# GadGadGad/Convolutional-KAN-for-Image-Classification

Measured on AMD Instinct MI355X. Metric: images/sec fwd+bwd KAN-VGG11 3x32x32 bs=256/GPU, higher is better.
Workload: dtype f32

## Files before the change

convolutional-kan-for-image-classification_amd/_lib.py:

```python
from __future__ import annotations

import ctypes as C
import os
from typing import Optional

_HERE = os.path.dirname(os.path.abspath(__file__))
LIB_PATH = os.environ.get("KANCONV_LIB") or os.path.join(_HERE, "libkanconv.so")

KAN_MAX_PLANES = 16
KAN_MAX_TABLE = 32
KAN_FP_WORDS = 192
BASIS_BSPLINE, BASIS_RBF, BASIS_CHEBY, BASIS_POLY, BASIS_FOURIER, BASIS_RELU, BASIS_GRAM = 0, 1, 2, 3, 4, 5, 6
ACT_NONE, ACT_IDENTITY, ACT_GELU, ACT_SILU, ACT_RELU, ACT_TANH, ACT_SIGMOID, ACT_GELU_TANH = -1, 0, 1, 2, 3, 4, 5, 6


class KanGeom(C.Structure):
    _fields_ = [(n, C.c_int) for n in ("B", "C", "H", "W", "O", "Ho", "Wo", "kh", "kw", "sh", "sw", "ph", "pw", "dh", "dw", "groups")] + \
               [("x_bstride", C.c_longlong), ("y_bstride", C.c_longlong)]


class KanBasis(C.Structure):
    _fields_ = [("kind", C.c_int), ("n_basis", C.c_int), ("order", C.c_int), ("act", C.c_int),
                ("p0", C.c_float), ("p1", C.c_float), ("table", C.c_float * KAN_MAX_TABLE), ("chan_table", C.c_void_p)]


class KanPlan(C.Structure):
    _fields_ = [(n, C.c_int) for n in ("P", "K", "IPC", "KC", "Kpad", "Opad", "fwd_splits", "bwd_data_splits", "bwd_weight_splits",
                                          "fwd_target", "bwd_data_target", "bwd_weight_target", "x_pm_wanted", "dz_pm_wanted", "bwd_weight_expanded", "row_blocks", "e_pm_wanted", "fwd_expanded", "fwd_halo", "bwd_weight_halo",
                                          "fwd_band", "bwd_weight_band")] + \
               [(n, C.c_longlong) for n in ("packed_weight_bytes", "bwd_data_weight_bytes", "fwd_slab_elems", "bwd_data_slab_elems",
                                            "bwd_weight_slab_elems", "e_pm_elems")]


class KanWavGeom(C.Structure):
    _fields_ = [(n, C.c_int) for n in ("B", "C", "H", "W", "O", "Ho", "Wo", "kh", "kw", "sh", "sw", "ph", "pw", "dh", "dw", "wavelet")] + \
               [("x_bstride", C.c_longlong), ("u_bstride", C.c_longlong)]


WAVELETS = {"mexican_hat": 0, "morlet": 1, "dog": 2, "meyer": 3, "shannon": 4}

_P, _I, _LL, _F, _D = C.c_void_p, C.c_int, C.c_longlong, C.c_float, C.c_double
_GP, _BP = C.POINTER(KanGeom), C.POINTER(KanBasis)
SIGNATURES = {
    "kan_version": (C.c_char_p, []),
    "kan_last_error": (C.c_char_p, []),
    "kan_plan": (_I, [_GP, _BP, C.POINTER(KanPlan)]),
    "kan_pack_weights": (_I, [_P, _P, _P, _P, _GP, _BP, _P]),
    "kan_pack_cacheable": (_I, [_GP, _BP]),
    "kan_pack_weights_cached": (_I, [_P, _P, _P, _P, _GP, _BP, _P, _I, _I, _I, _P]),
    "kan_conv_fwd": (_I, [_P, _P, _P, _P, _GP, _BP, _P, _P]),
    "kan_position_major": (_I, [_P, _P, _I, _I, _I, _LL, _P]),
    "kan_conv_bwd_data": (_I, [_P, _P, _P, _P, _P, _P, _GP, _BP, _P, _P]),
    "kan_conv_bwd_data_params": (_I, [_P, _P, _P, _P, _P, _P, _P, _GP, _BP, _P, _P]),
    "kan_conv_bwd_weight": (_I, [_P, _P, _P, _P, _GP, _BP, _P, _P, _P]),
    "kan_position_major_expanded": (_I, [_P, _P, _GP, _BP, _P]),
    "kan_conv_fwd_expanded": (_I, [_P, _P, _P, _GP, _BP, _P]),
    "kan_conv_bwd_weight_expanded": (_I, [_P, _P, _P, _GP, _BP, _P]),
    "kan_unpack_wgrad": (_I, [_P, _P, _P, _GP, _BP, _P]),
    "kan_slab_reduce": (_I, [_P, _I, _LL, _P, _I, _I, _I, _LL, _P]),
    "kan_instnorm_prelu_fwd": (_I, [_P, _I, _LL, _P, _P, _P, _P, _P, _P, _P, _I, _I, _I, _LL, _F, _I, _P]),
    "kan_instnorm_prelu_bwd": (_I, [_P, _P, _P, _P, _P, _P, _P, _P, _P, _P, _P, _I, _I, _I, _LL, _I, _P]),
    "kan_instnorm_prelu_pool_fwd": (_I, [_P, _I, _LL, _P, _P, _P, _P, _P, _P, _P, _P, _I, _I, _I, _I, _LL, _F, _I, _P]),
    "kan_instnorm_prelu_pool_bwd": (_I, [_P, _P, _P, _P, _P, _P, _P, _P, _P, _P, _P, _P, _I, _I, _I, _I, _LL, _I, _P]),
    "kan_instnorm_prelu_poolk_fwd": (_I, [_P, _I, _LL, _P, _P, _P, _P, _P, _P, _P, _P, _I, _I, _I, _I, _LL, _F, _I, _I, _I, _P]),
    "kan_instnorm_prelu_poolk_bwd": (_I, [_P, _P, _P, _P, _P, _P, _P, _P, _P, _P, _P, _P, _I, _I, _I, _I, _LL, _I, _I, _I, _P]),
    "kan_split_supported": (_I, [C.POINTER(KanGeom), C.POINTER(KanBasis)]),
    "kan_split_weight_bytes": (_LL, [C.POINTER(KanGeom), C.POINTER(KanBasis)]),
    "kan_split_pack_weights": (_I, [_P, _P, _P, C.POINTER(KanGeom), C.POINTER(KanBasis), _P]),
    "kan_conv_fwd_split": (_I, [_P, _P, _P, C.POINTER(KanGeom), C.POINTER(KanBasis), _P]),
    "kan_wav_fwd": (_I, [_P, _P, _P, _P, _P, C.POINTER(KanWavGeom), _P]),
    "kan_wav_bwd_input": (_I, [_P, _P, _P, _P, _P, _P, C.POINTER(KanWavGeom), _P]),
    "kan_wav_param_workspace": (_LL, [C.POINTER(KanWavGeom)]),
    "kan_wav_bwd_params": (_I, [_P, _P, _P, _P, _P, _P, _P, _P, _P, C.POINTER(KanWavGeom), _P]),
    "kan_adamw_step": (_I, [_P, _P, _P, _P, _LL, _D, _D, _D, _D, _D, _I, _F, _P]),
    "kan_adamw_step_segments": (_I, [_P, _P, _P, _P, _P, _P, _P, _P, _P, _I, _I, _D, _D, _D, _D, _D, _I, _F, _P]),
}

_lib: Optional[C.CDLL] = None

# ... 29 lines not shown
```

convolutional-kan-for-image-classification_amd/csrc/kanconv.hip:

```cpp
#include <hip/hip_runtime.h>
#include <cstdio>
#include <cstdlib>
#include <cstring>
#include <cmath>
#include <cstdint>
#include <type_traits>
#include "kanconv.h"
#include "kan_device.h"

#include "kan_common.h"
#include "kan_internal.h"

namespace {


thread_local char g_err[512] = "";
int fail(const char* fmt, const char* a = "") {
    snprintf(g_err, sizeof(g_err), fmt, a);
    return -1;
}
}
int kan_fail_msg(const char* fmt, const char* a) { return fail(fmt, a); }
namespace {

// ... 539 lines not shown
        for (int mi = 0; mi < 2; ++mi) {
#pragma unroll
            for (int r = 0; r < 16; ++r) {
                const int o = o_tile0 + w_o * 64 + mi * 32 + mfma_row(r, lane);
                if (o < g.O) zb[(size_t)o * HoWo] = acc[mi][ni][r];
            }
        }
    }
}

template <int M>
__device__ __forceinline__ void wave_reduce_scatter(float (&v)[M], int lane, int& idx, float& tot) {
    int base = 0;
    int m = M;
#pragma unroll
    for (int off = 32; off >= 1; off >>= 1) {
        if (m > 1) {
            const int h = m / 2;
            const bool up = (lane & off) != 0;
#pragma unroll
            for (int i = 0; i < M / 2; ++i) {
                if (i < h) {
                    const float keep = up ? v[h + i] : v[i], send = up ? v[i] : v[h + i];
                    v[i] = keep + __shfl_xor(send, off, 64);
                }
            }
            base += up ? h : 0;
            m = h;
        } else {
            v[0] += __shfl_xor(v[0], off, 64);
        }
    }
    idx = base; tot = v[0];
}

template <int KIND, int FAST, int RB = 0>
__global__ __launch_bounds__(256, 4) void k_conv_bwd_data(
    const float* __restrict__ dz, const float* __restrict__ x, const float* __restrict__ xn, const float* __restrict__ wd,
    float* __restrict__ dx, float* __restrict__ dxn, DevGeom g, DevBasis bs, int CH, int n_ct, int n_ob, int Opad16,
    int n_chunks, int chunks_per_split, long long slab_elems, unsigned dz_bytes, TilePerm perm, float* __restrict__ dpar) {
    constexpr int TP = 128, KD = 16, NT = 256;
    __shared__ __attribute__((aligned(16))) float smem[2 * 2 * KD * 128];
    __shared__ float sTab[KAN_MAX_TABLE];

    const int tid = threadIdx.x, lane = tid & 63;
    const int wave = __builtin_amdgcn_readfirstlane(tid >> 6);
    const int w_r = wave >> 1, w_p = wave & 1;
    const int HoWo = g.Ho * g.Wo, HW = g.H * g.W, P = bs.P;
    const int Min = g.B * HW;
    const BlockId blk = xcd_block_order(false);
    const int grp = blk.y / n_ct;
    const int px_tile0 = (perm.n ? (int)perm.idx[blk.x] : blk.x) * TP, ct = blk.y - grp * n_ct;
    const int ncol = n_ct * 128;
    const int pxl = (wave & 1) * 64 + lane, ol0 = wave >> 1;
    const bool idle_rows = (ct * 2 + w_r) * CH >= g.C;
    {
        const size_t xo = (size_t)grp * g.C * HW;
        x += xo; xn += xo; dx += xo; if (dxn) dxn += xo;
        dz += (size_t)grp * g.O * HoWo * (g.pix_major ? g.B : 1);
        wd += (size_t)grp * (g.kh * g.kw) * Opad16 * ncol;
    }

    if (tid < KAN_MAX_TABLE) sTab[tid] = bs.tab[tid];
    const int my_px = px_tile0 + (RB ? ((pxl >> 2) & 7) * 16 + (pxl >> 5) * 4 + (pxl & 3) : pxl);
    const bool pv = my_px < Min;
    int pb, ph_, pw_;
// ... 266 lines not shown
#pragma unroll
            for (int it = 0; it < NIT; ++it) {
                if (!((ok >> (half * NIT + it)) & 1u)) continue;
                const int cl = ol0 + 2 * it, c = (ct * 2 + half) * FCH + cl;
                const float xa = half == 0 ? xv[0][it] : xv[1][it];
                float dact;
                if (bs.act == KAN_ACT_SILU) {
                    const float sg = kan_rcp(1.0f + kan_exp2k(xa, -1.44269504088896340736f));
                    dact = sg * (1.0f + xa * (1.0f - sg));
                } else dact = kan_act_grad(bs.act, xa);
                float t = xa, chain = 1.0f;
                if (bs.order) {
                    t = kan_tanh_fast(xa);
                    chain = 1.0f - t * t;
                }
                const float* G = smem + (cl * FP) * TP + pxl;
                float Tm = bs.tab[0], Tc = bs.tab[1] * t + bs.tab[2], Dm = 0.f, Dc = bs.tab[1];
                float sb = 0.f;
#pragma unroll
                for (int k = 1; k < NB; ++k) {
                    sb += Dc * G[(1 + k) * TP];
                    if (k + 1 < NB) {
                        const float A = bs.tab[3 * k], B = bs.tab[3 * k + 1], Cc = bs.tab[3 * k + 2], sc = A * t + B;
                        const float Tn = sc * Tc + Cc * Tm, Dn = A * Tc + sc * Dc + Cc * Dm;
                        Tm = Tc; Tc = Tn; Dm = Dc; Dc = Dn;
                    }
                }
                dxs[(size_t)pb * g.xbs + (size_t)c * HW + (size_t)(ph_ * g.W + pw_)] = dact * G[0] + sb * chain;
            }
        }
        return;
    }
    if (FAST != 0) {
        constexpr int FP = 9, FCH = 7, NIT = (FCH + 1) / 2;
        float xv[2][NIT]; unsigned ok = 0;
#pragma unroll
        for (int half = 0; half < 2; ++half)
#pragma unroll
            for (int it = 0; it < NIT; ++it) {
                const int cl = ol0 + 2 * it, c = (ct * 2 + half) * FCH + cl;
                const bool v = cl < FCH && c < g.C && pv;
                xv[half][it] = v ? x[(size_t)pb * g.xbs + (size_t)c * HW + (size_t)(ph_ * g.W + pw_)] : 0.f;
                ok |= (v ? 1u : 0u) << (half * NIT + it);
            }
        const float hh = 0.5f * bs.inv_h;
#pragma unroll 1
        for (int half = 0; half < 2; ++half) {
            __syncthreads();
            if (w_r == half) {
#pragma unroll
                for (int mi = 0; mi < 2; ++mi)
#pragma unroll
                    for (int ni = 0; ni < 2; ++ni)
#pragma unroll
                        for (int r = 0; r < 16; ++r)
                            smem[(mi * 32 + mfma_row(r, lane)) * TP + w_p * 64 + ni * 32 + (lane & 31)] = acc[mi][ni][r];
            }
            __syncthreads();
#pragma unroll
            for (int it = 0; it < NIT; ++it) {
                if (!((ok >> (half * NIT + it)) & 1u)) continue;
                const int cl = ol0 + 2 * it, c = (ct * 2 + half) * FCH + cl;
                const float xa = half == 0 ? xv[0][it] : xv[1][it];
                float dact;
                if (FAST == 1) {
                    const float sg = kan_rcp(1.0f + kan_exp2k(xa, -1.44269504088896340736f));
                    dact = sg * (1.0f + xa * (1.0f - sg));
                } else dact = kan_act_grad(KAN_ACT_GELU, xa);
                const float* G = smem + (cl * FP) * TP + pxl;
                float sum = dact * G[0];
                if (xa >= bs.g0 && xa < bs.gN) {
                    const int i = min((int)((xa - bs.g0) * bs.inv_h), 10);
#ifdef KAN_EXACT_TRANSCENDENTALS
                    const double ihd = 1.0 / ((double)sTab[i + 1] - (double)sTab[i]), hd = 0.5 * ihd;
                    const double ud = fmin(fmax(((double)xa - (double)sTab[i]) * ihd, 0.0), 1.0), vd = 1.0 - ud, ud2 = ud * ud;
                    const float n0 = (float)(-hd * vd * vd), n1 = (float)(hd * (3.0 * ud2 - 4.0 * ud)), n2 = (float)(hd * (-3.0 * ud2 + 2.0 * ud + 1.0)), n3 = (float)(hd * ud2);
#else
                    const float u = fminf(fmaxf((xa - sTab[i]) * bs.inv_h, 0.f), 1.f), v = 1.f - u, u2 = u * u;
                    const float n0 = -hh * v * v, n1 = hh * (3.f * u2 - 4.f * u), n2 = hh * (-3.f * u2 + 2.f * u + 1.f), n3 = hh * u2;
#endif
                    const int j0 = i - 3;
                    sum += ((unsigned)j0 < 8u ? n0 * G[(1 + j0) * TP] : 0.f) + ((unsigned)(j0 + 1) < 8u ? n1 * G[(2 + j0) * TP] : 0.f)
                         + ((unsigned)(j0 + 2) < 8u ? n2 * G[(3 + j0) * TP] : 0.f) + ((unsigned)(j0 + 3) < 8u ? n3 * G[(4 + j0) * TP] : 0.f);
                }
                dxs[(size_t)pb * g.xbs + (size_t)c * HW + (size_t)(ph_ * g.W + pw_)] = sum;
            }
        }
        return;
    }
#pragma unroll 1
    for (int half = 0; half < 2; ++half) {
        __syncthreads();
        if (w_r == half) {
#pragma unroll
            for (int mi = 0; mi < 2; ++mi)
#pragma unroll
                for (int ni = 0; ni < 2; ++ni)
#pragma unroll
                    for (int r = 0; r < 16; ++r) {
                        int row = mi * 32 + mfma_row(r, lane);
                        int col = w_p * 64 + ni * 32 + (lane & 31);
                        smem[row * TP + col] = acc[mi][ni][r];
                    }
        }
        __syncthreads();
        for (int cl = ol0; cl < CH; cl += 2) {
            const int c = (ct * 2 + half) * CH + cl;
            if (c >= g.C || !pv) continue;
            const size_t idx = (size_t)pb * g.xbs + (size_t)c * HW + (size_t)(ph_ * g.W + pw_);
            const float xa = x[idx];
            const float xb = same_in ? xa : xn[idx];
            float s_base = 0.f, s_bas = 0.f;
            const float* Gc = smem + (cl * P) * TP + pxl;
            kan_planes_each<KIND, true>(bs, sTab, xa, xb, c, [&](int p, float d) {
                const float gv = Gc[p * TP];
                if (p < bs.hb) s_base += d * gv; else s_bas += d * gv;
            });
            if (split_out) { dxs[idx] = s_base; dxns[idx] = s_bas; }
            else dxs[idx] = s_base + s_bas;
        }
// ... 25 lines not shown
                const float xb = pv ? (same_in ? x : xn)[(size_t)pb * g.xbs + (size_t)c * HW + (size_t)(ph_ * g.W + pw_)] : 0.f;
                const float* lo = bs.ctab + (size_t)c * 2 * nb;
                if (2 * nb <= 16) {
                    float v[16];
#pragma unroll
                    for (int j = 0; j < 8; ++j) {
                        float vlo = 0.f, vhi = 0.f;
                        if (j < nb) {
                            const float gv = pv ? smem[(cl * P + hb + j) * TP + pxl] : 0.f;
                            const float x1 = fmaxf(xb - lo[j], 0.f), x2 = fmaxf(lo[nb + j] - xb, 0.f);
                            const float q2 = 2.0f * (x1 * x2 * rr) * rr;
                            vlo = -(q2 * x2) * gv; vhi = (q2 * x1) * gv;
                        }
                        v[j] = vlo; v[8 + j] = vhi;
                    }
                    int idx; float tot;
                    wave_reduce_scatter<16>(v, lane, idx, tot);
                    const int j = idx & 7;
                    if ((lane & 3) == 0 && j < nb) atomicAdd(dpar + (size_t)c * 2 * nb + (idx < 8 ? j : nb + j), tot);
                } else {
                    for (int j = 0; j < nb; ++j) {
                        const float gv = pv ? smem[(cl * P + hb + j) * TP + pxl] : 0.f;
                        const float x1 = fmaxf(xb - lo[j], 0.f), x2 = fmaxf(lo[nb + j] - xb, 0.f);
                        const float q2 = 2.0f * (x1 * x2 * rr) * rr;
                        float vlo = -(q2 * x2) * gv, vhi = (q2 * x1) * gv;
#pragma unroll
                        for (int off = 32; off > 0; off >>= 1) { vlo += __shfl_xor(vlo, off, 64); vhi += __shfl_xor(vhi, off, 64); }
                        if (lane == 0) { atomicAdd(dpar + (size_t)c * 2 * nb + j, vlo); atomicAdd(dpar + (size_t)c * 2 * nb + nb + j, vhi); }
                    }
                }
            }
        }
    }
}

template <int KIND, int FAST, int WR, int WC>
__global__ __launch_bounds__(WR * WC * 64, (WR * WC > 4 ? 2 : 4)) void k_conv_bwd_weight(
    const float* __restrict__ dz, const float* __restrict__ x, const float* __restrict__ xn, float* __restrict__ dwp,
    DevGeom g, DevBasis bs, int Krows, int Opad, int n_chunks, int chunks_per_split, long long slab_elems,
    unsigned x_bytes, unsigned dz_bytes, int tiles_o) {
    constexpr int TR = WR * 64, TO = WC * 64, NT = WR * WC * 64, KPX = 16;
    constexpr int MRG = KAN_PMAX;
    constexpr int LDE = TR + 2 * MRG + 1, LDZ = TO + 1;
    constexpr int IPP = NT / KPX;
    constexpr int UPF = TR / 128;
    constexpr int ZL = TO * KPX / NT;
    constexpr int MAXI = TR + 2;
    __shared__ float sE[2 * KPX * LDE];
    __shared__ float sZ[2 * KPX * LDZ];
    __shared__ int sItem[MAXI];
    __shared__ float sTab[KAN_MAX_TABLE];
    __shared__ float sDump[NT];

    const int tid = threadIdx.x, lane = tid & 63;
    const int wave = __builtin_amdgcn_readfirstlane(tid >> 6);
    const int w_r = wave / WC, w_c = wave % WC;
    const int HoWo = g.Ho * g.Wo, HW = g.H * g.W, T = g.kh * g.kw, P = FAST ? fast_planes(FAST) : bs.P;
    const int Mtot = g.B * HoWo, NI = g.C * T;
    const BlockId blk = xcd_block_order(!g.pix_major);
    const int grp = blk.y / tiles_o;
    const int k0 = blk.x * TR, o_tile0 = (blk.y - grp * tiles_o) * TO;
    {
        const int es = g.pix_major ? g.B : 1;
        const size_t xo = (size_t)grp * g.C * HW * es;
        x += xo; xn += xo;
        dz += (size_t)grp * g.O * HoWo * es;
// ... 1371 lines not shown
        if (best_cost < 0 || cost < best_cost) { best_cost = cost; best = t; best_ms = ms; }
    }
    *max_splits = best_ms;
    return best;
}
int live_taps_out(const KanGeom* g, int hw) {
    int n = 0;
    for (int tap = 0; tap < g->kh * g->kw; ++tap) {
        const int r = tap / g->kw, t = tap % g->kw, ho = hw / g->Wo, wo = hw % g->Wo;
        const int hi = ho * g->sh - g->ph + r * g->dh, wi = wo * g->sw - g->pw + t * g->dw;
        n += (hi >= 0 && hi < g->H && wi >= 0 && wi < g->W);
    }
    return n;
}
int live_taps_in(const KanGeom* g, int hw) {
    int n = 0;
    for (int tap = 0; tap < g->kh * g->kw; ++tap) {
        const int r = tap / g->kw, t = tap % g->kw, h = hw / g->W, w = hw % g->W;
        const int hn = h + g->ph - r * g->dh, wn = w + g->pw - t * g->dw;
        n += (hn >= 0 && wn >= 0 && hn % g->sh == 0 && wn % g->sw == 0 && hn / g->sh < g->Ho && wn / g->sw < g->Wo);
    }
    return n;
}
int live_positions_for_tap(const KanGeom* g, int tap) {
    int n = 0;
    for (int hw = 0; hw < g->Ho * g->Wo; ++hw) {
        const int r = tap / g->kw, t = tap % g->kw, ho = hw / g->Wo, wo = hw % g->Wo;
        const int hi = ho * g->sh - g->ph + r * g->dh, wi = wo * g->sw - g->pw + t * g->dw;
        n += (hi >= 0 && hi < g->H && wi >= 0 && wi < g->W);
    }
    return n;
}
struct BdCfg { int CH, tiles_c, tiles_p, n_ob, Opad32, chunks, splits; };
BdCfg bd_cfg(const KanGeom* g, const KanPlan& pl) {
    BdCfg c;
    c.CH = 64 / pl.P;
    c.tiles_c = ceil_div(g->C, 2 * c.CH);
    c.tiles_p = ceil_div((long long)g->B * g->H * g->W, 128);
    c.n_ob = ceil_div(g->O, 16);
    c.Opad32 = round_up(g->O, 32);
    c.chunks = g->kh * g->kw * c.n_ob;
    c.splits = pick_splits((long long)c.tiles_c * c.tiles_p * ngroups(g), c.chunks, 8, 4.0 * g->B * g->C * g->H * g->W * ngroups(g));
    return c;
}
bool pmdma_bwd_weight(const KanGeom* g, const KanBasis* b) {
    const int f = fast_variant(b);
    if (tuning_off("KAN_PMDMA") || !(f == 1 || f == 2 || f == 9 || f == 10)) return false;
    if (!want_pix_major(g, b, PM_BWD_WEIGHT)) return false;
    const int P = b->n_basis + (b->act != KAN_ACT_NONE);
    return (g->C * P) % 128 == 0 && g->B % 16 == 0 && round_up(g->O, 64) % 128 == 0 &&
           (long long)g->C * g->H * g->W * P * g->B * 4 < (1ll << 31);
}
bool pmdma_fwd(const KanGeom* g, const KanBasis* b) { return pmdma_fwd_shape(g, b) && want_pix_major(g, b, PM_FWD); }
bool halo_bwd_weight(const KanGeom* g, const KanBasis* b) {
    const int f = fast_variant(b);
    if (tuning_off("KAN_HALO_BW") || !(f == 1 || f == 2 || f == 9 || f == 10)) return false;
    if (g->kh != 3 || g->kw != 3 || g->sh != 1 || g->sw != 1 || g->dh != 1 || g->dw != 1 || g->ph != 1 || g->pw != 1) return false;
    if (round_up(g->O, 64) % 128 != 0 || g->C > 65535 / 81) return false;
    if (g->H != g->W) return false;
    if (g->W == 4) return !pmdma_bwd_weight(g, b) && g->B % 2 == 0 && g->C <= 256;
    return g->W == 16 || g->W == 8;
}
bool pm_bwd_weight(const KanGeom* g, const KanBasis* b) { return want_pix_major(g, b, PM_BWD_WEIGHT) && !halo_bwd_weight(g, b); }
struct BwHaloCfg { int R, nimg, spb, n_bands, tiles_r, tiles_o, splits, bands_per_split; };
BwHaloCfg bw_halo_cfg(const KanGeom* g, const KanPlan& pl) {
    BwHaloCfg c;
    c.R = g->W == 16 ? 4 : g->W;
    c.nimg = g->W == 4 ? 2 : 1;
    c.spb = c.nimg * c.R * g->W / 16;
    c.n_bands = g->B * (g->H / c.R) / c.nimg;
    c.tiles_r = ceil_div(pl.K, 128);
    c.tiles_o = pl.Opad / 128;
    const long long tiles = (long long)c.tiles_r * c.tiles_o * ngroups(g);
    const double slab_bytes = 4.0 * pl.K * pl.Opad * ngroups(g);
    int best = 1; double best_cost = -1;
// ... 27 lines not shown
    return !off && g->C == 1 && g->O <= 2 && T <= DW_T && T * P <= DW_MAX_TP;
}
int dw_weight_chunks(const KanGeom* g) {
    const long long total = (long long)g->B * g->Ho * g->Wo;
    int s = ceil_div(2048, ngroups(g));
    const int most = ceil_div(total, 256);
    if (s > most) s = most;
    if (s > 64) s = 64;
    return s < 1 ? 1 : s;
}

int make_plan(const KanGeom* g, const KanBasis* b, KanPlan* pl) {
    if (int rc = check(g, b)) return rc;
    const int T = g->kh * g->kw;
    pl->P = b->n_basis + (b->act != KAN_ACT_NONE);
    pl->K = g->C * T * pl->P;
    {
        int i18 = 18 / pl->P, i16 = 16 / pl->P;
        if (i18 > 4) i18 = 4;
        if (i16 > 4) i16 = 4;
        const bool use18 = (long long)i18 * pl->P * 16 > (long long)i16 * pl->P * 18;
        pl->KC = use18 ? 18 : 16;
        pl->IPC = use18 ? i18 : i16;
        if (pl->P >= 10 && pl->P <= 12) { pl->KC = 12; pl->IPC = 1; }
        if (halo_fwd(g, b)) { pl->KC = 2 * pl->P; pl->IPC = 2; }
    }
    pl->Kpad = ceil_div(g->C * T, pl->IPC) * pl->KC;
    KanBandCfg band;
    const bool use_band = band_fwd(g, b, &band);
    if (use_band) { pl->KC = band.NPLE; pl->IPC = band.NG; pl->Kpad = band.n_steps * band.NPLE; }
    pl->Opad = round_up(g->O, 64);
    const int G = ngroups(g);
    pl->packed_weight_bytes = (long long)G * pl->Kpad * pl->Opad * 4;
    BdCfg bd = bd_cfg(g, *pl);
    pl->bwd_data_weight_bytes = (long long)G * T * bd.Opad32 * bd.tiles_c * 128 * 4;
    pl->fwd_slab_elems = (long long)g->B * g->y_bstride;
    pl->bwd_data_slab_elems = (long long)g->B * g->x_bstride;
    pl->bwd_weight_slab_elems = (long long)G * pl->K * pl->Opad;
    pl->fwd_splits = use_band ? band.fwd_splits : fwd_cfg(g, b, *pl).splits;
    pl->fwd_band = use_band ? 1 : 0;
    pl->bwd_weight_band = (use_band && band.bw_ok && !want_pix_major(g, b, PM_BWD_WEIGHT) && !tuning_off("KAN_BAND_BW")) ? 1 : 0;
    pl->bwd_data_splits = bd.splits;
    pl->bwd_weight_splits = halo_bwd_weight(g, b) ? bw_halo_cfg(g, *pl).splits : bw_cfg(g, b, *pl).splits;
    if (pl->bwd_weight_band) {
        pl->bwd_weight_splits = band.bw_splits;
        pl->bwd_weight_slab_elems = (long long)G * pl->Kpad * pl->Opad;
    }
    pl->x_pm_wanted = ((want_pix_major(g, b, PM_FWD) && !pmdma_fwd(g, b)) || (pm_bwd_weight(g, b) && !pmdma_bwd_weight(g, b))) ? 1 : 0;
    pl->dz_pm_wanted = (want_pix_major(g, b, PM_BWD_DATA) || pm_bwd_weight(g, b)) ? 1 : 0;
    pl->fwd_target = pl->bwd_data_target = pl->bwd_weight_target = 0;
    pl->fwd_halo = halo_fwd(g, b) ? 1 : 0;
    pl->bwd_weight_halo = (halo_bwd_weight(g, b) && !pl->bwd_weight_band) ? 1 : 0;
    pl->e_pm_wanted = 0; pl->fwd_expanded = 0; pl->bwd_weight_expanded = 0; pl->e_pm_elems = 0;
    pl->row_blocks = (rowblk_fwd(g, b, *pl) ? 1 : 0) | (rowblk_bwd_data(g, b) ? 2 : 0);
    if (dw_direct(g, b)) {
        pl->fwd_halo = pl->bwd_weight_halo = pl->fwd_band = pl->bwd_weight_band = 0;
        pl->fwd_splits = pl->bwd_data_splits = 1;
        pl->bwd_weight_splits = dw_weight_chunks(g);
        pl->x_pm_wanted = pl->dz_pm_wanted = 0;
        pl->bwd_data_weight_bytes = pl->packed_weight_bytes;
        return 0;
    }
    if (want_pix_major(g, b, PM_FWD)) {
        LiveClass cls[16]; const int plane = g->Ho * g->Wo; FwdCfg fc = fwd_cfg(g, b, *pl);
        const long long tiles_per_pos = (long long)ceil_div(g->B, fc.TP) * fc.tiles_o * G;
        for (int hw = 0; hw < plane; ++hw) cls[hw] = LiveClass{tiles_per_pos, live_taps_out(g, hw) * ceil_div(g->C, pl->IPC)};
        pl->fwd_target = pick_target_steps(cls, plane, 8, 4.0 * g->B * g->O * g->Ho * g->Wo * G, &pl->fwd_splits, fc.slots);
// ... 140 lines not shown
        for (int i = threadIdx.x; i < (n >> 2); i += 256) {
            float4 P = ((float4*)p)[i], G = ((const float4*)g)[i], M = ((float4*)m)[i], V = ((float4*)v)[i];
            adam1(P.x, G.x, M.x, V.x, a); adam1(P.y, G.y, M.y, V.y, a); adam1(P.z, G.z, M.z, V.z, a); adam1(P.w, G.w, M.w, V.w, a);
            ((float4*)p)[i] = P; ((float4*)m)[i] = M; ((float4*)v)[i] = V;
        }
        const int t = (n & ~3) + threadIdx.x;
        if (t < n) adam1(p[t], g[t], m[t], v[t], a);
    } else {
        for (int i = threadIdx.x; i < n; i += 256) adam1(p[i], g[i], m[i], v[i], a);
    }
}

AdamArgs adam_args(double lr, double beta1, double beta2, double eps, double weight_decay, int step, float grad_scale) {
    const double bc1 = 1.0 - pow(beta1, (double)step), bc2 = 1.0 - pow(beta2, (double)step);
    AdamArgs a;
    a.decay = (float)(1.0 - lr * weight_decay);
    a.w1 = (float)(1.0 - beta1); a.b2 = (float)beta2; a.w2 = (float)(1.0 - beta2);
    a.gscale = grad_scale; a.inv_bc2_sqrt = (float)(1.0 / sqrt(bc2)); a.eps = (float)eps; a.neg_step = (float)(-lr / bc1);
    return a;
}

#include "wavkan.inc"

}

extern "C" {

const char* kan_version(void) { return "kanconv 0.5 (gfx950, fp32 MFMA 32x32x2, halo forward, 128/256-output tiles)"; }
const char* kan_last_error(void) { return g_err; }

int kan_plan(const KanGeom* geom, const KanBasis* basis, KanPlan* plan) {
    if (!plan) return fail("null plan");
    return make_plan(geom, basis, plan);
}

static bool pack_needs_clear(const KanGeom* g, const KanPlan& pl) {
    if (pl.fwd_band) return pl.KC != pl.IPC * pl.P || g->C % pl.IPC != 0;
    return pl.KC != pl.IPC * pl.P || (g->C * g->kh * g->kw) % pl.IPC != 0;
}

static int pack_weights_impl(const float* w_base, const float* w_basis, float* wp, float* wd, const KanGeom* g, const KanBasis* b,
                             const unsigned long long* fp, int fp_cur, void* stream) {
    KanPlan pl;
    if (int rc = make_plan(g, b, &pl)) return rc;
    const int hb = b->act != KAN_ACT_NONE;
    if ((hb && !w_base) || !w_basis || !wp) return fail("null weight pointer");
    hipStream_t st = (hipStream_t)stream;
    const int T = g->kh * g->kw, NI = g->C * T, G = ngroups(g);
    const long long wp_gs = (long long)pl.Kpad * pl.Opad;
    PackGeo q = pack_geo(g, b, pl, false);
    if (fp && (pack_needs_clear(g, pl) || dw_direct(g, b))) return fail("cached packing is not offered for this geometry (kan_pack_cacheable)");
    if (pl.KC != pl.IPC * pl.P || (pl.fwd_band && pack_needs_clear(g, pl))) {
        if (hipMemsetAsync(wp, 0, (size_t)pl.packed_weight_bytes, st) != hipSuccess) return fail("memset failed");
    } else if (!pl.fwd_band && NI % pl.IPC != 0) {
        if (G > 1) {
            if (hipMemsetAsync(wp, 0, (size_t)pl.packed_weight_bytes, st) != hipSuccess) return fail("memset failed");
        } else {
            size_t off = (size_t)(pl.Kpad - pl.KC) * pl.Opad;
            if (hipMemsetAsync(wp + off, 0, (size_t)pl.KC * pl.Opad * 4, st) != hipSuccess) return fail("memset failed");
        }
    }
    const int nb_base = hb ? ceil_div(g->C * T, 32) : 0;
    const int tiles_x = nb_base + ceil_div(g->C * b->n_basis * T, 32), tiles_y = pl.Opad / 32;
    const long long n_tiles = (long long)tiles_x * tiles_y;
    const long long cap = fp ? 1024 : 4096;
    dim3 grid((unsigned)(n_tiles < cap ? n_tiles : cap), 1, G);
    hipLaunchKernelGGL(k_pack, grid, dim3(256), 0, st, w_base, w_basis, wp, q, nb_base, wp_gs, tiles_x, tiles_y, fp, fp_cur);
    if (wd && dw_direct(g, b)) {
        if (hipMemcpyAsync(wd, wp, (size_t)pl.packed_weight_bytes, hipMemcpyDeviceToDevice, st) != hipSuccess) return fail("memcpy failed");
    } else if (wd) {
        BdCfg c = bd_cfg(g, pl);
        const int bx = c.tiles_c * 4, by = c.Opad32 / 32 * G;
        const long long nt = (long long)bx * by;
        const long long capd = fp ? 128 : 1024;
        dim3 gd((unsigned)(nt < capd ? nt : capd), 1, T);
        hipLaunchKernelGGL(k_pack_bwd_data, gd, dim3(256), 0, st, (const float*)wp, wd, q, c.CH, c.tiles_c, c.Opad32, wp_gs, bx, by, fp, fp_cur);
    }
    return launch_ok("pack");
}

int kan_pack_weights(const float* w_base, const float* w_basis, float* wp, float* wd, const KanGeom* g, const KanBasis* b, void* stream) {
    return pack_weights_impl(w_base, w_basis, wp, wd, g, b, nullptr, 0, stream);
}

int kan_pack_cacheable(const KanGeom* g, const KanBasis* b) {
    KanPlan pl;
    if (make_plan(g, b, &pl)) return 0;
    if ((long long)g->O * g->C * (b->n_basis + 1) * g->kh * g->kw >= (1ll << 31)) return 0;
    return (!pack_needs_clear(g, pl) && !dw_direct(g, b) && ngroups(g) == 1) ? 1 : 0;
}

int kan_pack_weights_cached(const float* w_base, const float* w_basis, float* wp, float* wd, const KanGeom* g, const KanBasis* b,
                            unsigned long long* ring, int cur, int force, int sample_stride, void* stream) {
    static_assert(KAN_FP_WORDS == 3 * FP_LANES, "ring size");
    if (!ring || cur < 0 || cur > 2 || sample_stride < 1) return fail("bad fingerprint ring arguments");
    if (!kan_pack_cacheable(g, b)) return fail("cached packing is not offered for this geometry (kan_pack_cacheable)");
    const int hb = b->act != KAN_ACT_NONE;
    if ((hb && !w_base) || !w_basis) return fail("null weight pointer");
    if (((size_t)w_basis & 15) || (hb && ((size_t)w_base & 15))) return fail("cached packing needs 16-byte aligned weight tensors");
    const int T = g->kh * g->kw;
    const long long na = hb ? (long long)g->O * g->C * T : 0, nbs = (long long)g->O * g->C * b->n_basis * T;
    const long long groups4 = ((na + 3) / 4 + (nbs + 3) / 4 + sample_stride - 1) / sample_stride;
    long long blocks = (groups4 + 256 * 8 - 1) / (256 * 8); if (blocks > 4096) blocks = 4096; if (blocks < 1) blocks = 1;
    hipLaunchKernelGGL(k_fingerprint, dim3((unsigned)blocks), dim3(256), 0, (hipStream_t)stream, hb ? w_base : w_basis, (unsigned)na, w_basis,
// ... 158 lines not shown
}

int kan_conv_bwd_data_params(const float* dz, const float* x, const float* xn, const float* wd, float* dx, float* dxn, float* dparams,
                             const KanGeom* g, const KanBasis* b, const float* dz_pm, void* stream) {
    if (!dparams) return fail("null dparams");
    if (b && b->kind != KAN_BASIS_RELU && b->kind != KAN_BASIS_GRAM) return fail("kan_conv_bwd_data_params: only the ReLU-KAN and GRAM bases accumulate parameter gradients in this launch");
    if (g && b && dw_direct(g, b)) return fail("kan_conv_bwd_data_params: depthwise layers take the weight-gradient route");
    return conv_bwd_data_impl(dz, x, xn, wd, dx, dxn, dparams, g, b, dz_pm, stream);
}

static int conv_bwd_data_impl(const float* dz, const float* x, const float* xn, const float* wd, float* dx, float* dxn, float* dpar,
                              const KanGeom* g, const KanBasis* b, const float* dz_pm, void* stream) {
    KanPlan pl;
    if (int rc = make_plan(g, b, &pl)) return rc;
    if (!dz || !x || !xn || !wd || !dx) return fail("null tensor pointer");
    if ((b->kind == KAN_BASIS_RELU || b->kind == KAN_BASIS_GRAM) && !b->chan_table) return fail("ReLU / Gram bases need their device parameter table (chan_table)");
    if (!dxn && x != xn) return fail("dxn is required when xn != x");
    if (dw_direct(g, b)) {
        DevGeom dgd = dev_geom(g); DevBasis dbd = dev_basis(b);
        dim3 grid(ceil_div((long long)g->B * g->H * g->W, 256), ngroups(g));
#define KAN_DWD(KIND) hipLaunchKernelGGL((k_dw_bwd_data<KIND>), grid, dim3(256), 0, (hipStream_t)stream, dz, x, xn, wd, dx, dxn, dgd, dbd, pl.Opad, pl.IPC, pl.KC, pl.Kpad)
        switch (b->kind) {
            case KAN_BASIS_BSPLINE: KAN_DWD(KAN_BASIS_BSPLINE); break;
            case KAN_BASIS_RBF: KAN_DWD(KAN_BASIS_RBF); break;
            case KAN_BASIS_POLY: KAN_DWD(KAN_BASIS_POLY); break;
            case KAN_BASIS_FOURIER: KAN_DWD(KAN_BASIS_FOURIER); break;
            case KAN_BASIS_RELU: KAN_DWD(KAN_BASIS_RELU); break;
            case KAN_BASIS_GRAM: KAN_DWD(KAN_BASIS_GRAM); break;
            default: KAN_DWD(KAN_BASIS_CHEBY); break;
        }
#undef KAN_DWD
        return launch_ok("dw_bwd_data");
    }
    BdCfg c = bd_cfg(g, pl);
    DevGeom dg = dev_geom(g);
    dg.pix_major = (dz_pm && want_pix_major(g, b, PM_BWD_DATA)) ? 1 : 0;
    if (dg.pix_major) dz = dz_pm;
    DevBasis db = dev_basis(b);
    hipStream_t st = (hipStream_t)stream;
    if ((long long)c.tiles_c * ngroups(g) > 65535) return fail("groups * channel tiles exceed the grid limit");
    dim3 grid(c.tiles_p, c.tiles_c * ngroups(g), pl.bwd_data_splits);
    int cps = dg.pix_major ? pl.bwd_data_target : ceil_div(c.chunks, pl.bwd_data_splits);
    TilePerm perm; perm.n = 0;
    if (dg.pix_major && c.tiles_p <= PERM_MAX) {
        int w[PERM_MAX];
        for (int t = 0; t < c.tiles_p; ++t) {
            const int hw = (int)(((long long)t * 128) / g->B);
            w[t] = ceil_div(live_taps_in(g, hw < g->H * g->W ? hw : 0) * c.n_ob, cps > 0 ? cps : 1);
        }
        perm = balance_tiles(w, c.tiles_p);
    }
#define KAN_BD(KIND) KAN_BD2(KIND, 0)
#define KAN_BD2(KIND, FAST) \
    hipLaunchKernelGGL((k_conv_bwd_data<KIND, FAST>), grid, dim3(256), 0, st, dz, x, xn, wd, dx, dxn, dg, db, c.CH, c.tiles_c, c.n_ob, c.Opad32, c.chunks, cps, pl.bwd_data_slab_elems, (unsigned)((long long)g->B * g->y_bstride * 4), perm, dpar)
    const int fv = fast_variant(b);
    const int fast = (fv == 3 || fv == 8) ? ((x != xn && dxn) ? fv : 0) : ((x == xn && !dxn) ? fv : 0);
    const bool rb = !dg.pix_major && rowblk_bwd_data(g, b);
#define KAN_BD3(KIND, FAST) \
    hipLaunchKernelGGL((k_conv_bwd_data<KIND, FAST, 1>), grid, dim3(256), 0, st, dz, x, xn, wd, dx, dxn, dg, db, c.CH, c.tiles_c, c.n_ob, c.Opad32, c.chunks, cps, pl.bwd_data_slab_elems, (unsigned)((long long)g->B * g->y_bstride * 4), perm, dpar)
    if (fast == 1 && rb) KAN_BD3(KAN_BASIS_BSPLINE, 1);
    else if (fast == 2 && rb) KAN_BD3(KAN_BASIS_BSPLINE, 2);
    else if (fast == 1) KAN_BD2(KAN_BASIS_BSPLINE, 1);
    else if (fast == 2) KAN_BD2(KAN_BASIS_BSPLINE, 2);
    else if (fast == 3) KAN_BD2(KAN_BASIS_RBF, 3);
    else if (fast == 8) KAN_BD2(KAN_BASIS_RBF, 8);
    else if (fast == 4) KAN_BD2(KAN_BASIS_CHEBY, 4);
    else if (fast == 5) KAN_BD2(KAN_BASIS_CHEBY, 5);
    else if (fast == 6) KAN_BD2(KAN_BASIS_POLY, 6);
// ... 366 lines not shown
```

include/kanconv.h:

```cpp
#ifndef KANCONV_H
#define KANCONV_H

#ifdef __cplusplus
extern "C" {
#endif

#define KAN_MAX_PLANES 16
#define KAN_MAX_TABLE  32
#define KAN_FP_WORDS   192

enum { KAN_BASIS_BSPLINE = 0, KAN_BASIS_RBF = 1, KAN_BASIS_CHEBY = 2, KAN_BASIS_POLY = 3, KAN_BASIS_FOURIER = 4, KAN_BASIS_RELU = 5, KAN_BASIS_GRAM = 6 };
enum { KAN_ACT_NONE = -1, KAN_ACT_IDENTITY = 0, KAN_ACT_GELU = 1, KAN_ACT_SILU = 2, KAN_ACT_RELU = 3,
       KAN_ACT_TANH = 4, KAN_ACT_SIGMOID = 5, KAN_ACT_GELU_TANH = 6 };

typedef struct KanGeom {
    int B, C, H, W;
    int O, Ho, Wo;
    int kh, kw, sh, sw, ph, pw, dh, dw;
    int groups;
    long long x_bstride;
    long long y_bstride;
} KanGeom;

typedef struct KanBasis {
    int kind, n_basis, order, act;
    float p0, p1;
    float table[KAN_MAX_TABLE];
    const float* chan_table;
} KanBasis;

typedef struct KanPlan {
    int P;
    int K;
    int IPC, KC;
    int Kpad, Opad;
    int fwd_splits;
    int bwd_data_splits;
    int bwd_weight_splits;
    int fwd_target, bwd_data_target, bwd_weight_target;
    int x_pm_wanted, dz_pm_wanted;
    int bwd_weight_expanded;
    int row_blocks;
    int e_pm_wanted, fwd_expanded;
    int fwd_halo, bwd_weight_halo;
    int fwd_band, bwd_weight_band;
    long long packed_weight_bytes;
    long long bwd_data_weight_bytes;
    long long fwd_slab_elems;
    long long bwd_data_slab_elems;
    long long bwd_weight_slab_elems;
    long long e_pm_elems;
} KanPlan;

const char* kan_version(void);
const char* kan_last_error(void);

int kan_plan(const KanGeom* geom, const KanBasis* basis, KanPlan* plan);

int kan_pack_weights(const float* w_base, const float* w_basis, float* wp, float* wd,
                     const KanGeom* geom, const KanBasis* basis, void* stream);

int kan_pack_cacheable(const KanGeom* geom, const KanBasis* basis);
int kan_pack_weights_cached(const float* w_base, const float* w_basis, float* wp, float* wd,
                            const KanGeom* geom, const KanBasis* basis, unsigned long long* ring, int cur, int force,
                            int sample_stride, void* stream);

int kan_conv_fwd(const float* x, const float* xn, const float* wp, float* z,
                 const KanGeom* geom, const KanBasis* basis, const float* x_pm, void* stream);

int kan_position_major(const float* src, float* dst, int B, int Cn, int HW, long long bstride, void* stream);

int kan_conv_bwd_data(const float* dz, const float* x, const float* xn, const float* wd,
                      float* dx, float* dxn,
                      const KanGeom* geom, const KanBasis* basis, const float* dz_pm, void* stream);

int kan_conv_bwd_data_params(const float* dz, const float* x, const float* xn, const float* wd, float* dx, float* dxn, float* dparams,
                             const KanGeom* geom, const KanBasis* basis, const float* dz_pm, void* stream);

int kan_conv_bwd_weight(const float* dz, const float* x, const float* xn, float* dwp,
                        const KanGeom* geom, const KanBasis* basis, const float* x_pm, const float* dz_pm, void* stream);

int kan_position_major_expanded(const float* x, float* e_pm, const KanGeom* geom, const KanBasis* basis, void* stream);
int kan_conv_fwd_expanded(const float* e_pm, const float* wp, float* z, const KanGeom* geom, const KanBasis* basis, void* stream);
int kan_conv_bwd_weight_expanded(const float* dz_pm, const float* e_pm, float* dwp,
                                 const KanGeom* geom, const KanBasis* basis, void* stream);

int kan_unpack_wgrad(const float* dwp, float* dw_base, float* dw_basis,
                     const KanGeom* geom, const KanBasis* basis, void* stream);

int kan_slab_reduce(const float* slabs, int n_slabs, long long slab_elems, float* out,
// ... 60 lines not shown
```

Measured before the change: 17210.

## Add halo-tiled bwd-data kernel for 4x4 3x3 KAN conv layers

Adds a specialized backward-data kernel for 3x3 stride-1 convolutions on 4x4 spatial maps. For each output-channel block it loads a zero-padded halo of dz for 8 images into LDS once, then reuses that halo across all nine taps via shifted LDS addressing, with double-buffered weight loads. The existing B-spline epilogue is factored into a shared helper, and the split count is adjusted so the output-channel blocks divide evenly across splits. This only affects the small late VGG layers, so its share of total fwd+bwd time is limited, and it adds code complexity and LDS pressure.

```diff
diff --git a/convolutional-kan-for-image-classification_amd/_lib.py b/convolutional-kan-for-image-classification_amd/_lib.py
--- a/convolutional-kan-for-image-classification_amd/_lib.py
+++ b/convolutional-kan-for-image-classification_amd/_lib.py
@@ -45,6 +45,7 @@
     "kan_version": (C.c_char_p, []),
     "kan_last_error": (C.c_char_p, []),
     "kan_plan": (_I, [_GP, _BP, C.POINTER(KanPlan)]),
+    "kan_bwd_data_kernel": (_I, [_GP, _BP]),
     "kan_pack_weights": (_I, [_P, _P, _P, _P, _GP, _BP, _P]),
     "kan_pack_cacheable": (_I, [_GP, _BP]),
     "kan_pack_weights_cached": (_I, [_P, _P, _P, _P, _GP, _BP, _P, _I, _I, _I, _P]),
diff --git a/convolutional-kan-for-image-classification_amd/csrc/kanconv.hip b/convolutional-kan-for-image-classification_amd/csrc/kanconv.hip
--- a/convolutional-kan-for-image-classification_amd/csrc/kanconv.hip
+++ b/convolutional-kan-for-image-classification_amd/csrc/kanconv.hip
@@ -595,6 +595,68 @@
         }
     }
     idx = base; tot = v[0];
+}
+
+template <int FAST>
+__device__ __forceinline__ void bd_epilogue_bspline(const f32x16 (&acc)[2][2], float* smem, const float* sTab, const DevGeom& g, const DevBasis& bs,
+                                                    const float* __restrict__ x, float* __restrict__ dxs, int ct, int ol0, int w_r, int w_p,
+                                                    int lane, int pxl, bool pv, int pb, int ph_, int pw_) {
+    constexpr int TP = 128;
+    const int HW = g.H * g.W;
+    constexpr int FP = 9, FCH = 7, NIT = (FCH + 1) / 2;
+    float xv[2][NIT]; unsigned ok = 0;
+#pragma unroll
+    for (int half = 0; half < 2; ++half)
+#pragma unroll
+        for (int it = 0; it < NIT; ++it) {
+            const int cl = ol0 + 2 * it, c = (ct * 2 + half) * FCH + cl;
+            const bool v = cl < FCH && c < g.C && pv;
+            xv[half][it] = v ? x[(size_t)pb * g.xbs + (size_t)c * HW + (size_t)(ph_ * g.W + pw_)] : 0.f;
+            ok |= (v ? 1u : 0u) << (half * NIT + it);
+        }
+    const float hh = 0.5f * bs.inv_h;
+#pragma unroll 1
+    for (int half = 0; half < 2; ++half) {
+        __syncthreads();
+        if (w_r == half) {
+#pragma unroll
+            for (int mi = 0; mi < 2; ++mi)
+#pragma unroll
+                for (int ni = 0; ni < 2; ++ni)
+#pragma unroll
+                    for (int r = 0; r < 16; ++r)
+                        smem[(mi * 32 + mfma_row(r, lane)) * TP + w_p * 64 + ni * 32 + (lane & 31)] = acc[mi][ni][r];
+        }
+        __syncthreads();
+#pragma unroll
+        for (int it = 0; it < NIT; ++it) {
+            if (!((ok >> (half * NIT + it)) & 1u)) continue;
+            const int cl = ol0 + 2 * it, c = (ct * 2 + half) * FCH + cl;
+            const float xa = half == 0 ? xv[0][it] : xv[1][it];
+            float dact;
+            if (FAST == 1) {
+                const float sg = kan_rcp(1.0f + kan_exp2k(xa, -1.44269504088896340736f));
+                dact = sg * (1.0f + xa * (1.0f - sg));
+            } else dact = kan_act_grad(KAN_ACT_GELU, xa);
+            const float* G = smem + (cl * FP) * TP + pxl;
+            float sum = dact * G[0];
+            if (xa >= bs.g0 && xa < bs.gN) {
+                const int i = min((int)((xa - bs.g0) * bs.inv_h), 10);
+#ifdef KAN_EXACT_TRANSCENDENTALS
+                const double ihd = 1.0 / ((double)sTab[i + 1] - (double)sTab[i]), hd = 0.5 * ihd;
+                const double ud = fmin(fmax(((double)xa - (double)sTab[i]) * ihd, 0.0), 1.0), vd = 1.0 - ud, ud2 = ud * ud;
+                const float n0 = (float)(-hd * vd * vd), n1 = (float)(hd * (3.0 * ud2 - 4.0 * ud)), n2 = (float)(hd * (-3.0 * ud2 + 2.0 * ud + 1.0)), n3 = (float)(hd * ud2);
+#else
+                const float u = fminf(fmaxf((xa - sTab[i]) * bs.inv_h, 0.f), 1.f), v = 1.f - u, u2 = u * u;
+                const float n0 = -hh * v * v, n1 = hh * (3.f * u2 - 4.f * u), n2 = hh * (-3.f * u2 + 2.f * u + 1.f), n3 = hh * u2;
+#endif
+                const int j0 = i - 3;
+                sum += ((unsigned)j0 < 8u ? n0 * G[(1 + j0) * TP] : 0.f) + ((unsigned)(j0 + 1) < 8u ? n1 * G[(2 + j0) * TP] : 0.f)
+                     + ((unsigned)(j0 + 2) < 8u ? n2 * G[(3 + j0) * TP] : 0.f) + ((unsigned)(j0 + 3) < 8u ? n3 * G[(4 + j0) * TP] : 0.f);
+            }
+            dxs[(size_t)pb * g.xbs + (size_t)c * HW + (size_t)(ph_ * g.W + pw_)] = sum;
+        }
+    }
 }
 
 template <int KIND, int FAST, int RB = 0>
@@ -927,60 +989,7 @@
         return;
     }
     if (FAST != 0) {
-        constexpr int FP = 9, FCH = 7, NIT = (FCH + 1) / 2;
-        float xv[2][NIT]; unsigned ok = 0;
-#pragma unroll
-        for (int half = 0; half < 2; ++half)
-#pragma unroll
-            for (int it = 0; it < NIT; ++it) {
-                const int cl = ol0 + 2 * it, c = (ct * 2 + half) * FCH + cl;
-                const bool v = cl < FCH && c < g.C && pv;
-                xv[half][it] = v ? x[(size_t)pb * g.xbs + (size_t)c * HW + (size_t)(ph_ * g.W + pw_)] : 0.f;
-                ok |= (v ? 1u : 0u) << (half * NIT + it);
-            }
-        const float hh = 0.5f * bs.inv_h;
-#pragma unroll 1
-        for (int half = 0; half < 2; ++half) {
-            __syncthreads();
-            if (w_r == half) {
-#pragma unroll
-                for (int mi = 0; mi < 2; ++mi)
-#pragma unroll
-                    for (int ni = 0; ni < 2; ++ni)
-#pragma unroll
-                        for (int r = 0; r < 16; ++r)
-                            smem[(mi * 32 + mfma_row(r, lane)) * TP + w_p * 64 + ni * 32 + (lane & 31)] = acc[mi][ni][r];
-            }
-            __syncthreads();
-#pragma unroll
-            for (int it = 0; it < NIT; ++it) {
-                if (!((ok >> (half * NIT + it)) & 1u)) continue;
-                const int cl = ol0 + 2 * it, c = (ct * 2 + half) * FCH + cl;
-                const float xa = half == 0 ? xv[0][it] : xv[1][it];
-                float dact;
-                if (FAST == 1) {
-                    const float sg = kan_rcp(1.0f + kan_exp2k(xa, -1.44269504088896340736f));
-                    dact = sg * (1.0f + xa * (1.0f - sg));
-                } else dact = kan_act_grad(KAN_ACT_GELU, xa);
-                const float* G = smem + (cl * FP) * TP + pxl;
-                float sum = dact * G[0];
-                if (xa >= bs.g0 && xa < bs.gN) {
-                    const int i = min((int)((xa - bs.g0) * bs.inv_h), 10);
-#ifdef KAN_EXACT_TRANSCENDENTALS
-                    const double ihd = 1.0 / ((double)sTab[i + 1] - (double)sTab[i]), hd = 0.5 * ihd;
-                    const double ud = fmin(fmax(((double)xa - (double)sTab[i]) * ihd, 0.0), 1.0), vd = 1.0 - ud, ud2 = ud * ud;
-                    const float n0 = (float)(-hd * vd * vd), n1 = (float)(hd * (3.0 * ud2 - 4.0 * ud)), n2 = (float)(hd * (-3.0 * ud2 + 2.0 * ud + 1.0)), n3 = (float)(hd * ud2);
-#else
-                    const float u = fminf(fmaxf((xa - sTab[i]) * bs.inv_h, 0.f), 1.f), v = 1.f - u, u2 = u * u;
-                    const float n0 = -hh * v * v, n1 = hh * (3.f * u2 - 4.f * u), n2 = hh * (-3.f * u2 + 2.f * u + 1.f), n3 = hh * u2;
-#endif
-                    const int j0 = i - 3;
-                    sum += ((unsigned)j0 < 8u ? n0 * G[(1 + j0) * TP] : 0.f) + ((unsigned)(j0 + 1) < 8u ? n1 * G[(2 + j0) * TP] : 0.f)
-                         + ((unsigned)(j0 + 2) < 8u ? n2 * G[(3 + j0) * TP] : 0.f) + ((unsigned)(j0 + 3) < 8u ? n3 * G[(4 + j0) * TP] : 0.f);
-                }
-                dxs[(size_t)pb * g.xbs + (size_t)c * HW + (size_t)(ph_ * g.W + pw_)] = sum;
-            }
-        }
+        bd_epilogue_bspline<FAST>(acc, smem, sTab, g, bs, x, dxs, ct, ol0, w_r, w_p, lane, pxl, pv, pb, ph_, pw_);
         return;
     }
 #pragma unroll 1
@@ -1072,6 +1081,160 @@
             }
         }
     }
+}
+
+template <int FAST, int W, int R, int NIMG>
+__global__ __launch_bounds__(256, 4) void k_conv_bwd_data_halo(
+    const float* __restrict__ dz, const float* __restrict__ x, const float* __restrict__ wd, float* __restrict__ dx,
+    DevGeom g, DevBasis bs, int n_ct, int n_ob, int Opad32, int obs_per_split, long long slab_elems, unsigned dz_bytes) {
+    constexpr int TP = 128, KD = 16, T = 9, CH = 7;
+    constexpr bool RB = (R * W == 16 && NIMG * W == 32);
+    constexpr int HW_ = W + 2, HIMG = (R + 2) * HW_, HALO = NIMG * HIMG;
+    constexpr int ZST = HALO, NCH = (ZST + 63) / 64;
+    constexpr int SW = 2 * KD * 128, NS = SW + KD * ZST > 64 * 128 ? SW + KD * ZST : 64 * 128;
+    static_assert(RB && NIMG * R * W == TP && ZST >= 64, "tile shape: 4x4 planes, 8 images");
+    __shared__ __attribute__((aligned(16))) float smem[NS];
+    __shared__ float sTab[KAN_MAX_TABLE];
+    float* const sZ = smem + SW;
+
+    const int tid = threadIdx.x, lane = tid & 63;
+    const int wave = __builtin_amdgcn_readfirstlane(tid >> 6);
+    const int w_r = wave >> 1, w_p = wave & 1;
+    const int HW = g.H * g.W, Min = g.B * HW;
+    const BlockId blk = xcd_block_order(false);
+    const int grp = blk.y / n_ct;
+    const int px_tile0 = blk.x * TP, ct = blk.y - grp * n_ct;
+    const int ncol = n_ct * 128;
+    const int pxl = (wave & 1) * 64 + lane, ol0 = wave >> 1;
+    const bool idle_rows = (ct * 2 + w_r) * CH >= g.C;
+    {
+        const size_t xo = (size_t)grp * g.C * HW;
+        x += xo; dx += xo;
+        dz += (size_t)grp * g.O * HW;
+        wd += (size_t)grp * T * Opad32 * ncol;
+    }
+    if (tid < KAN_MAX_TABLE) sTab[tid] = bs.tab[tid];
+    const int my_px = px_tile0 + ((pxl >> 2) & 7) * 16 + (pxl >> 5) * 4 + (pxl & 3);
+    const bool pv = my_px < Min;
+    const int pb = my_px / HW, phw = my_px - pb * HW, ph_ = phw / W, pw_ = phw - ph_ * W;
+
+    const int b0 = px_tile0 / HW, h0 = (px_tile0 - b0 * HW) / W;
+    unsigned zoff[NCH];
+#pragma unroll
+    for (int j = 0; j < NCH; ++j) {
+        const int cell = (j + 1 < NCH ? j * 64 : ZST - 64) + lane;
+        const int img = cell / HIMG, rc = cell - img * HIMG, hr = rc / HW_, hc = rc - hr * HW_;
+        const int b = b0 + img, h = h0 - 1 + hr, w = hc - 1;
+        const bool ok = b < g.B && hr < R + 2 && (unsigned)h < (unsigned)g.H && (unsigned)w < (unsigned)W;
+        zoff[j] = ok ? ((unsigned)b * (unsigned)g.ybs + (unsigned)(h * W + w)) * 4u : KAN_OOB;
+    }
+    const kan_rsrc dz_rs = make_rsrc(dz, dz_bytes);
+    const unsigned row_bytes = (unsigned)HW * 4u;
+    auto issue_halo = [&](int ob) {
+        const int o0 = ob * KD;
+#pragma unroll
+        for (int i = 0; i < KD / 4; ++i) {
+            const int o = wave + 4 * i;
+            const bool live = o0 + o < g.O;
+            const unsigned so = live ? (unsigned)(o0 + o) * row_bytes : 0u;
+#pragma unroll
+            for (int j = 0; j < NCH; ++j)
+                __builtin_amdgcn_raw_ptr_buffer_load_lds(dz_rs, (__attribute__((address_space(3))) void*)(sZ + o * ZST + (j + 1 < NCH ? j * 64 : ZST - 64)), 4,
+                                                         (int)(live ? zoff[j] : KAN_OOB), (int)so, 0, 0);
+        }
+    };
+    const unsigned wlane = (unsigned)((lane >> 5) * ncol + (lane & 31) * 4) * 4u;
+    auto issue_w = [&](int ob, int k, int buf) {
+        int rowA, rowB;
+        if (RB && k >= 3) { const int t = (k - 3) >> 1, h = (k - 3) & 1; rowA = t * Opad32 + ob * KD + 8 * h; rowB = rowA + 6 * Opad32; }
+        else { rowA = (RB ? 3 + k : k) * Opad32 + ob * KD; rowB = rowA + 8; }
+        float* dW = smem + buf * (KD * 128);
+#pragma unroll
+        for (int j = 0; j < 2; ++j) {
+            const int blk2 = j * 4 + wave;
+            const int row = (blk2 < 4 ? rowA : rowB) + (blk2 & 3) * 2;
+            glds16((const float*)((const char*)(wd + (size_t)row * ncol + ct * 128) + wlane), dW + blk2 * 256);
+        }
+    };
+
+    const int kh2 = lane >> 5;
+    unsigned vb[2];
+#pragma unroll
+    for (int q = 0; q < 2; ++q) {
+        const int n = w_p * 64 + q * 32 + (lane & 31);
+        const int row = n / (NIMG * W), rem = n - row * (NIMG * W), img = rem / W, col = rem - img * W;
+        vb[q] = lds_addr(sZ + kh2 * ZST + img * HIMG + (row + 1) * HW_ + (col + 1));
+    }
+    const unsigned aw0 = lds_addr(smem + kh2 * 128 + w_r * 64 + (lane & 31));
+
+    f32x16 acc[2][2];
+#pragma unroll
+    for (int a = 0; a < 2; ++a)
+#pragma unroll
+        for (int b = 0; b < 2; ++b)
+#pragma unroll
+            for (int r = 0; r < 16; ++r) acc[a][b][r] = 0.f;
+
+    const int ob0 = blk.z * obs_per_split, ob1 = min(n_ob, ob0 + obs_per_split);
+    if (ob0 < ob1) { issue_halo(ob0); issue_w(ob0, 0, 0); }
+    int buf = 0;
+    for (int ob = ob0; ob < ob1; ++ob) {
+#pragma unroll 1
+        for (int k = 0; k < T; ++k) {
+            asm volatile("s_waitcnt vmcnt(0)" ::: "memory");
+            __syncthreads();
+            if (k + 1 < T) issue_w(ob, k + 1, buf ^ 1);
+            else if (ob + 1 < ob1) issue_w(ob + 1, 0, buf ^ 1);
+            const bool mixed = RB && k >= 3;
+            int sA, sB;
+            if (mixed) {
+                const int t = (k - 3) >> 1, h = (k - 3) & 1;
+                sA = (HW_ + 1 - t + 8 * h * ZST) * 4; sB = sA - 2 * HW_ * 4;
+            } else {
+                const int tap = RB ? 3 + k : k, r = tap / 3, t = tap - 3 * r;
+                sA = ((1 - r) * HW_ + (1 - t)) * 4; sB = sA + 8 * ZST * 4;
+            }
+            const bool l0b = !(mixed && w_p == 0), l1a = !(mixed && w_p == 1);
+            const unsigned aw = aw0 + (unsigned)buf * (KD * 128 * 4);
+            const unsigned bA0 = vb[0] + (unsigned)sA, bA1 = vb[1] + (unsigned)sA;
+            const unsigned bB0 = RB ? vb[0] + (unsigned)sB : bA0, bB1 = RB ? vb[1] + (unsigned)sB : bA1;
+#define KAN_HB_OFF(kk) ((RB ? 2 * ((kk) & 3) : 2 * (kk)) * ZST * 4)
+            const bool last = k == T - 1 && ob + 1 < ob1;
+            if (!idle_rows) {
+                float fa[2][2], fb[2][2];
+                LDS_READ4H(fa[0][0], fa[0][1], fb[0][0], fb[0][1], aw, bA0, bA1, 0, 32 * 4, 0);
+#pragma unroll
+                for (int kk = 0; kk < 8; ++kk) {
+                    const int c_ = kk & 1, n_ = c_ ^ 1;
+                    if (kk + 1 < 8) {
+                        LDS_READ4H(fa[n_][0], fa[n_][1], fb[n_][0], fb[n_][1], aw, kk + 1 < 4 ? bA0 : bB0, kk + 1 < 4 ? bA1 : bB1,
+                                   (2 * (kk + 1)) * 128 * 4, (2 * (kk + 1)) * 128 * 4 + 128, KAN_HB_OFF(kk + 1));
+                        LDS_WAIT4(fa[c_][0], fa[c_][1], fb[c_][0], fb[c_][1], 4);
+                    } else {
+                        LDS_WAIT4(fa[c_][0], fa[c_][1], fb[c_][0], fb[c_][1], 0);
+                        if (last) {
+                            asm volatile("s_barrier" ::: "memory");
+                            issue_halo(ob + 1);
+                        }
+                    }
+                    if (kk < 4 || l0b) {
+                        acc[0][0] = MFMA32(fa[c_][0], fb[c_][0], acc[0][0]);
+                        acc[1][0] = MFMA32(fa[c_][1], fb[c_][0], acc[1][0]);
+                    }
+                    if (kk >= 4 || l1a) {
+                        acc[0][1] = MFMA32(fa[c_][0], fb[c_][1], acc[0][1]);
+                        acc[1][1] = MFMA32(fa[c_][1], fb[c_][1], acc[1][1]);
+                    }
+                }
+            } else if (last) {
+                asm volatile("s_barrier" ::: "memory");
+                issue_halo(ob + 1);
+            }
+#undef KAN_HB_OFF
+            buf ^= 1;
+        }
+    }
+    bd_epilogue_bspline<FAST>(acc, smem, sTab, g, bs, x, dx + (size_t)blk.z * slab_elems, ct, ol0, w_r, w_p, lane, pxl, pv, pb, ph_, pw_);
 }
 
 template <int KIND, int FAST, int WR, int WC>
@@ -2509,7 +2672,14 @@
     return n;
 }
 struct BdCfg { int CH, tiles_c, tiles_p, n_ob, Opad32, chunks, splits; };
-BdCfg bd_cfg(const KanGeom* g, const KanPlan& pl) {
+bool halo_bwd_data(const KanGeom* g, const KanBasis* b) {
+    const int f = fast_variant(b);
+    if (tuning_off("KAN_HALO_BD") || !(f == 1 || f == 2)) return false;
+    if (g->kh != 3 || g->kw != 3 || g->sh != 1 || g->sw != 1 || g->dh != 1 || g->dw != 1 || g->ph != 1 || g->pw != 1) return false;
+    if ((g->C & 1) || want_pix_major(g, b, PM_BWD_DATA)) return false;
+    return g->H == 4 && g->W == 4 && rowblk_bwd_data(g, b);
+}
+BdCfg bd_cfg(const KanGeom* g, const KanBasis* b, const KanPlan& pl) {
     BdCfg c;
     c.CH = 64 / pl.P;
     c.tiles_c = ceil_div(g->C, 2 * c.CH);
@@ -2518,6 +2688,10 @@
     c.Opad32 = round_up(g->O, 32);
     c.chunks = g->kh * g->kw * c.n_ob;
     c.splits = pick_splits((long long)c.tiles_c * c.tiles_p * ngroups(g), c.chunks, 8, 4.0 * g->B * g->C * g->H * g->W * ngroups(g));
+    if (halo_bwd_data(g, b)) {
+        const int obps = ceil_div(c.n_ob, c.splits < c.n_ob ? c.splits : c.n_ob);
+        c.splits = ceil_div(c.n_ob, obps);
+    }
     return c;
 }
 bool pmdma_bwd_weight(const KanGeom* g, const KanBasis* b) {
@@ -2611,7 +2785,7 @@
     pl->Opad = round_up(g->O, 64);
     const int G = ngroups(g);
     pl->packed_weight_bytes = (long long)G * pl->Kpad * pl->Opad * 4;
-    BdCfg bd = bd_cfg(g, *pl);
+    BdCfg bd = bd_cfg(g, b, *pl);
     pl->bwd_data_weight_bytes = (long long)G * T * bd.Opad32 * bd.tiles_c * 128 * 4;
     pl->fwd_slab_elems = (long long)g->B * g->y_bstride;
     pl->bwd_data_slab_elems = (long long)g->B * g->x_bstride;
@@ -2818,6 +2992,13 @@
 int kan_plan(const KanGeom* geom, const KanBasis* basis, KanPlan* plan) {
     if (!plan) return fail("null plan");
     return make_plan(geom, basis, plan);
+}
+
+int kan_bwd_data_kernel(const KanGeom* geom, const KanBasis* basis) {
+    KanPlan pl;
+    if (make_plan(geom, basis, &pl)) return -1;
+    if (dw_direct(geom, basis)) return 0;
+    return halo_bwd_data(geom, basis) ? 2 : rowblk_bwd_data(geom, basis) ? 1 : 0;
 }
 
 static bool pack_needs_clear(const KanGeom* g, const KanPlan& pl) {
@@ -2855,7 +3036,7 @@
     if (wd && dw_direct(g, b)) {
         if (hipMemcpyAsync(wd, wp, (size_t)pl.packed_weight_bytes, hipMemcpyDeviceToDevice, st) != hipSuccess) return fail("memcpy failed");
     } else if (wd) {
-        BdCfg c = bd_cfg(g, pl);
+        BdCfg c = bd_cfg(g, b, pl);
         const int bx = c.tiles_c * 4, by = c.Opad32 / 32 * G;
         const long long nt = (long long)bx * by;
         const long long capd = fp ? 128 : 1024;
@@ -3080,8 +3261,21 @@
 #undef KAN_DWD
         return launch_ok("dw_bwd_data");
     }
-    BdCfg c = bd_cfg(g, pl);
+    BdCfg c = bd_cfg(g, b, pl);
     DevGeom dg = dev_geom(g);
+    if (halo_bwd_data(g, b) && x == xn && !dxn) {
+        if ((long long)c.tiles_c * ngroups(g) > 65535) return fail("groups * channel tiles exceed the grid limit");
+        const DevBasis dbh = dev_basis(b);
+        const int obps = ceil_div(c.n_ob, pl.bwd_data_splits);
+        const unsigned dz_bytes = (unsigned)((long long)g->B * g->y_bstride * 4);
+        dim3 gridh(c.tiles_p, c.tiles_c * ngroups(g), pl.bwd_data_splits);
+#define KAN_BDH(F, WV, RV, NV) hipLaunchKernelGGL((k_conv_bwd_data_halo<F, WV, RV, NV>), gridh, dim3(256), 0, (hipStream_t)stream, dz, x, wd, dx, dg, dbh, \
+                                                  c.tiles_c, c.n_ob, c.Opad32, obps, pl.bwd_data_slab_elems, dz_bytes)
+        const int fv = fast_variant(b);
+        if (fv == 1) KAN_BDH(1, 4, 4, 8); else KAN_BDH(2, 4, 4, 8);
+#undef KAN_BDH
+        return launch_ok("conv_bwd_data_halo");
+    }
     dg.pix_major = (dz_pm && want_pix_major(g, b, PM_BWD_DATA)) ? 1 : 0;
     if (dg.pix_major) dz = dz_pm;
     DevBasis db = dev_basis(b);
diff --git a/include/kanconv.h b/include/kanconv.h
--- a/include/kanconv.h
+++ b/include/kanconv.h
@@ -56,6 +56,8 @@
 const char* kan_last_error(void);
 
 int kan_plan(const KanGeom* geom, const KanBasis* basis, KanPlan* plan);
+
+int kan_bwd_data_kernel(const KanGeom* geom, const KanBasis* basis);
 
 int kan_pack_weights(const float* w_base, const float* w_basis, float* wp, float* wd,
                      const KanGeom* geom, const KanBasis* basis, void* stream);
```

Result: no change. 17210, median of 6 (+0.0%).
